# Samsung/tf-fast-rnnt

Hardware: AMD Instinct MI355X
Metric: rnnt_loss_pruned_fwd_bwd_throughput (higher is better)
Workload: dtype f32; 1 GPU; c3: rnnt_loss_pruned fwd+bwd step, B=32/GPU T=1000 S=200 C=500 s_range=5, regular, full boundary, first pass rnnt_loss_simple; global_batch=32, am_pruned=broadcast view

## Files before the change

### tf-fast-rnnt_amd/csrc/prune.hip

```cpp
#include "ftr_common.h"
#include "launch.h"
#include "act_math.h"
#include <cstdlib>
#include <limits.h>

namespace ftr {
namespace {

__device__ __forceinline__ int wave_incl_min_scan(int v, int lane) {
#pragma unroll
  for (int off = 1; off < 64; off <<= 1) {
    const int t = __shfl_up(v, off, 64);
    if (lane >= off) v = min(v, t);
  }
  return v;
}

__global__ void cummin_kernel(const int32_t* __restrict__ in, int32_t* __restrict__ out, int rows, int cols) {
  const int lane = threadIdx.x & 63;
  const int row = blockIdx.x * (blockDim.x >> 6) + (threadIdx.x >> 6);
  if (row >= rows) return;
  const int32_t* src = in + (size_t)row * cols;
  int32_t* dst = out + (size_t)row * cols;
  int carry = INT_MAX;
// ... 13 lines not shown
  const int t = blockIdx.x * blockDim.x + threadIdx.x;
  const int b = blockIdx.y;
  if (t >= T) return;
  const int S1 = S + 1;
  const int nwin = S1 - r + 1;
  const float* pyc = py_grad + (size_t)b * S1 * T + t;
  const float* pxc = px_grad + (size_t)b * S * T1 + t;
  float lead = 0.0f, lag = 0.0f;
  for (int s = 0; s < r; ++s) lead = lead + pyc[(size_t)s * T];
  int best = 0;
  float bestv = 0.0f;
  constexpr int CHK = 16;
  float ld[2][CHK], lg[2][CHK], xv[2][CHK];
  auto fetch = [&](int c0, float (&l)[CHK], float (&g)[CHK], float (&x)[CHK]) {
#pragma unroll
    for (int u = 0; u < CHK; ++u) {
      const int s0 = c0 + u;
      const bool more = s0 + 1 < nwin;
      l[u] = more ? pyc[(size_t)(s0 + r) * T] : 0.0f;
      g[u] = more ? pyc[(size_t)s0 * T] : 0.0f;
      x[u] = (s0 > 0 && s0 < nwin) ? pxc[(size_t)(s0 - 1) * T1] : 0.0f;
    }
  };
  auto consume = [&](int c0, const float (&l)[CHK], const float (&g)[CHK], const float (&x)[CHK]) {
#pragma unroll
    for (int u = 0; u < CHK; ++u) {
      const int s0 = c0 + u;
      if (s0 < nwin) {
        const float blk = lead - lag;
        const float fin = blk - x[u];
        if (s0 == 0 || fin > bestv) { best = s0; bestv = fin; }
        if (s0 + 1 < nwin) {
          lead = lead + l[u];
          lag = lag + g[u];
        }
      }
    }
  };
  fetch(0, ld[0], lg[0], xv[0]);
  for (int c0 = 0; c0 < nwin; c0 += 2 * CHK) {
    if (c0 + CHK < nwin) fetch(c0 + CHK, ld[1], lg[1], xv[1]);
    consume(c0, ld[0], lg[0], xv[0]);
    if (c0 + CHK < nwin) {
      if (c0 + 2 * CHK < nwin) fetch(c0 + 2 * CHK, ld[0], lg[0], xv[0]);
      consume(c0 + CHK, ld[1], lg[1], xv[1]);
    }
  }
  const int se = boundary[4 * b + 2], te = boundary[4 * b + 3];
  int pad = se - r + 1;
  if (pad < 0) pad = 0;
  s_begin[(size_t)b * T + t] = (t < te - 1) ? best : pad;
}

constexpr int kSplitQ = 64;
__global__ __launch_bounds__(512) void prune_argmax_split_kernel(const float* __restrict__ px_grad, const float* __restrict__ py_grad,
                                                                 const int32_t* __restrict__ boundary, int32_t* __restrict__ s_begin,
                                                                 int B, int S, int T, int T1, int r) {
  __shared__ float st_lead[64], st_lag[64], st_bestv[64];
  __shared__ int st_best[64];
  const int lane = threadIdx.x & 63, wave = threadIdx.x >> 6, NW = blockDim.x >> 6;
  const int t = blockIdx.x * 64 + lane;
  const int b = blockIdx.y;
  const bool live = t < T;
  const int tc = live ? t : T - 1;
  const int S1 = S + 1;
  const int nwin = S1 - r + 1;
  const float* pyc = py_grad + (size_t)b * S1 * T + tc;
  const float* pxc = px_grad + (size_t)b * S * T1 + tc;
  constexpr int Q = kSplitQ;
  const int NC = (nwin + Q - 1) / Q;
  float n[Q], g[Q], x[Q];
  auto fetch = [&](int c) {
    const int c0 = c * Q;
#pragma unroll
    for (int u = 0; u < Q; ++u) {
      const int s0 = c0 + u;
      const bool more = s0 + 1 < nwin;
      n[u] = more ? pyc[(size_t)(s0 + r) * T] : 0.0f;
      g[u] = more ? pyc[(size_t)s0 * T] : 0.0f;
      x[u] = (s0 > 0 && s0 < nwin) ? pxc[(size_t)(s0 - 1) * T1] : 0.0f;
    }
  };
  if (wave < NC) fetch(wave);
  float lead = 0.0f, lag = 0.0f, bestv = 0.0f;
  int best = 0;
  if (wave == 0)
    for (int s = 0; s < r; ++s) lead = lead + pyc[(size_t)s * T];
  for (int c = 0; c < NC; ++c) {
    if (c % NW == wave) {
      if (c > 0) { lead = st_lead[lane]; lag = st_lag[lane]; bestv = st_bestv[lane]; best = st_best[lane]; }
      const int c0 = c * Q;
#pragma unroll
      for (int u = 0; u < Q; ++u) {
        const int s0 = c0 + u;
        if (s0 < nwin) {
          const float blk = lead - lag;
          const float fin = blk - x[u];
          if (s0 == 0 || fin > bestv) { best = s0; bestv = fin; }
          if (s0 + 1 < nwin) {
            lead = lead + n[u];
            lag = lag + g[u];
          }
        }
      }
      if (c + 1 < NC) { st_lead[lane] = lead; st_lag[lane] = lag; st_bestv[lane] = bestv; st_best[lane] = best; }
      if (c + NW < NC) fetch(c + NW);
      if (c + 1 == NC && live) {
        const int se = boundary[4 * b + 2], te = boundary[4 * b + 3];
        int pad = se - r + 1;
        if (pad < 0) pad = 0;
        s_begin[(size_t)b * T + t] = (t < te - 1) ? best : pad;
      }
    }
    if (c + 1 < NC) __syncthreads();
  }
}

constexpr int kPruneChk = 64;
template <int R>
__global__ __launch_bounds__(64) void prune_argmax_once_kernel(const float* __restrict__ px_grad, const float* __restrict__ py_grad,
                                         const int32_t* __restrict__ boundary, int32_t* __restrict__ s_begin,
                                         int B, int S, int T, int T1) {
  const int t = blockIdx.x * blockDim.x + threadIdx.x;
  const int b = blockIdx.y;
  if (t >= T) return;
  const int S1 = S + 1;
  const int nwin = S1 - R + 1;
  const float* pyc = py_grad + (size_t)b * S1 * T + t;
  const float* pxc = px_grad + (size_t)b * S * T1 + t;
  constexpr int CHK = kPruneChk;
  float carry[R];
  float lead = 0.0f, lag = 0.0f;
#pragma unroll
  for (int s = 0; s < R; ++s) { carry[s] = pyc[(size_t)s * T]; }
#pragma unroll
  for (int s = 0; s < R; ++s) lead = lead + carry[s];
  int best = 0;
  float bestv = 0.0f;
  float nv[2][CHK], xv[2][CHK];
  auto fetch = [&](int c0, float (&n)[CHK], float (&x)[CHK]) {
#pragma unroll
    for (int u = 0; u < CHK; ++u) {
      const int s0 = c0 + u;
      n[u] = (s0 + 1 < nwin) ? pyc[(size_t)(s0 + R) * T] : 0.0f;
      x[u] = (s0 > 0 && s0 < nwin) ? pxc[(size_t)(s0 - 1) * T1] : 0.0f;
    }
  };
  auto consume = [&](int c0, const float (&n)[CHK], const float (&x)[CHK]) {
#pragma unroll
    for (int u = 0; u < CHK; ++u) {
      const int s0 = c0 + u;
      const float g = (u < R) ? carry[u < R ? u : 0] : n[u >= R ? u - R : 0];
      if (s0 < nwin) {
        const float blk = lead - lag;
        const float fin = blk - x[u];
        if (s0 == 0 || fin > bestv) { best = s0; bestv = fin; }
        if (s0 + 1 < nwin) {
          lead = lead + n[u];
          lag = lag + g;
        }
      }
    }
#pragma unroll
    for (int i = 0; i < R; ++i) carry[i] = n[CHK - R + i];
  };
  fetch(0, nv[0], xv[0]);
  for (int c0 = 0; c0 < nwin; c0 += 2 * CHK) {
    if (c0 + CHK < nwin) fetch(c0 + CHK, nv[1], xv[1]);
    consume(c0, nv[0], xv[0]);
    if (c0 + CHK < nwin) {
      if (c0 + 2 * CHK < nwin) fetch(c0 + 2 * CHK, nv[0], xv[0]);
      consume(c0 + CHK, nv[1], xv[1]);
    }
  }
  const int se = boundary[4 * b + 2], te = boundary[4 * b + 3];
  int pad = se - R + 1;
  if (pad < 0) pad = 0;
  s_begin[(size_t)b * T + t] = (t < te - 1) ? best : pad;
}

__device__ __forceinline__ int wave_incl_suffix_min(int v, int lane) {
#pragma unroll
  for (int off = 1; off < 64; off <<= 1) {
    const int t = __shfl_down(v, off, 64);
    if (lane + off < 64) v = min(v, t);
  }
  return v;
}

__global__ void prune_adjust_kernel(const int32_t* __restrict__ s_begin, int32_t* __restrict__ ranges, int B,
                                    int T, int r_out, int r_con) {
  const int lane = threadIdx.x & 63;
  const int b = blockIdx.x * (blockDim.x >> 6) + (threadIdx.x >> 6);
  if (b >= B) return;
  constexpr int PER = 16, SB = 64 * PER;
  const int32_t* x = s_begin + (size_t)b * T;
  int carry1 = INT_MAX, carry2 = INT_MAX;
  for (int base = ((T - 1) / SB) * SB; base >= 0; base -= SB) {
    const int t0 = base + lane * PER;
    int v[PER];
#pragma unroll
    for (int i = 0; i < PER; ++i) v[i] = (t0 + i < T) ? x[t0 + i] : INT_MAX;
#pragma unroll
    for (int i = PER - 2; i >= 0; --i) v[i] = min(v[i], v[i + 1]);
    int incl = wave_incl_suffix_min(v[0], lane);
    int right = __shfl_down(incl, 1, 64);
    right = (lane == 63) ? carry1 : min(right, carry1);
    carry1 = min(__shfl(incl, 0, 64), carry1);
#pragma unroll
    for (int i = 0; i < PER; ++i) {
      const int t = t0 + i;
      v[i] = (t < T) ? -(min(v[i], right) - (r_con - 1) * t) : INT_MAX;
    }
#pragma unroll
    for (int i = PER - 2; i >= 0; --i) v[i] = min(v[i], v[i + 1]);
    incl = wave_incl_suffix_min(v[0], lane);
    right = __shfl_down(incl, 1, 64);
    right = (lane == 63) ? carry2 : min(right, carry2);
    carry2 = min(__shfl(incl, 0, 64), carry2);
#pragma unroll
    for (int i = 0; i < PER; ++i) {
      const int t = t0 + i;
      if (t < T) {
        const int z = max(min(v[i], right), 0);
        const int sb = -(z - (r_con - 1) * t);
        int32_t* dst = ranges + ((size_t)b * T + t) * r_out;
        for (int k = 0; k < r_out; ++k) dst[k] = sb + k;
      }
    }
  }
}

template <bool VEC>
__global__ __launch_bounds__(128) void do_pruning_kernel(const float* __restrict__ am, const float* __restrict__ lm,
                                                         const int32_t* __restrict__ ranges, float* __restrict__ am_p,
                                                         float* __restrict__ lm_p, int T, int S1, int C, int r) {
  const bool copy_am = am_p != nullptr;
  size_t bt = blockIdx.x;
  if ((gridDim.x & 7u) == 0) bt = (size_t)(blockIdx.x & 7u) * (gridDim.x >> 3) + (blockIdx.x >> 3);
  const size_t b = bt / T;
  const int32_t* rg = ranges + bt * r;
  const float* lmb = lm + b * S1 * C;
  float* ao = am_p + bt * r * C;
  float* lo = lm_p + bt * r * C;
  if (VEC) {
    const int n4 = C >> 2;
    const f4u* arow = reinterpret_cast<const f4u*>(am + bt * C);
    for (int c4 = threadIdx.x; c4 < n4; c4 += 128) {
      f4 a = {0.0f, 0.0f, 0.0f, 0.0f};
      if (copy_am) a = arow[c4];
      for (int k0 = 0; k0 < r; k0 += 8) {
        f4 l[8];
#pragma unroll
        for (int u = 0; u < 8; ++u)
          if (k0 + u < r) l[u] = reinterpret_cast<const f4u*>(lmb + (size_t)min(max(rg[k0 + u], 0), S1 - 1) * C)[c4];
#pragma unroll
        for (int u = 0; u < 8; ++u)
          if (k0 + u < r) {
            if (copy_am) __builtin_nontemporal_store(a, reinterpret_cast<f4u*>(ao + (size_t)(k0 + u) * C) + c4);
            __builtin_nontemporal_store(l[u], reinterpret_cast<f4u*>(lo + (size_t)(k0 + u) * C) + c4);
          }
      }
    }
  } else {
    for (int c = threadIdx.x; c < C; c += 128) {
      const float a = copy_am ? am[bt * C + c] : 0.0f;
      for (int k = 0; k < r; ++k) {
        if (copy_am) ao[(size_t)k * C + c] = a;
        lo[(size_t)k * C + c] = lmb[(size_t)min(max(rg[k], 0), S1 - 1) * C + c];
      }
    }
  }
// ... 1325 lines not shown
    constexpr auto kernel = joiner_act_bwd_lm_kernel<E, ACT, decltype(v)::value>;
    const int rcl = reserve_lds<kernel>(lds, "do_pruning_bwd", LdsText::reserve_why);
    if (rcl != FTR_OK) return rcl;
    hipLaunchKernelGGL(kernel, dim3(S1, B), dim3(64), lds, st, g, y, ranges, d_lm, T, S1, C, r);
    return check_launch("do_pruning_bwd_lm");
  });
}
template <typename E, int ACT>
int joiner_act_bwd_routes(const E* g, const E* y, const int32_t* ranges, E* d_am, E* d_lm, int B, int T, int S1, int C, int r,
                          void* ws, size_t ws_bytes, hipStream_t st) {
  if ((size_t)B * T * C == 0) return FTR_OK;
  const bool vec = bwd_vec4(C, g, y, d_am, d_lm);
  if (!vec || r <= 0) return joiner_act_bwd_generic<E, ACT>(g, y, ranges, d_am, d_lm, B, T, S1, C, r, vec, st);
  const size_t need = do_pruning_bwd_workspace_bytes(B, T, S1, C, r);
  if (!ws || ws_bytes < need || (reinterpret_cast<uintptr_t>(ws) & 15) != 0) {
    set_error("do_pruning_bwd_ws: workspace of %zu bytes (16-byte aligned) required, got %zu", need, ws_bytes);
    return FTR_ERR_INVALID_ARG;
  }
  const int seg = seg_frames(B, T);
  const int nseg = (T + seg - 1) / seg;
  float* partial = reinterpret_cast<float*>(ws);
  int4* meta = reinterpret_cast<int4*>(partial + (size_t)B * nseg * (2 * (size_t)r) * C);
  const size_t lds = sizeof(int) * (size_t)seg;
  if (r > kSegMaxR || lds > 60 * 1024 || (size_t)B * nseg * (2 * (size_t)r) >= 0x7fffffffull || (size_t)B * T * r >= 0x7fffffffull)
    return joiner_act_bwd_generic<E, ACT>(g, y, ranges, d_am, d_lm, B, T, S1, C, r, vec, st);
  dispatch_range<1, kSegMaxR>(r, [&](auto rr) {
    hipLaunchKernelGGL((joiner_act_bwd_seg_kernel<E, ACT, decltype(rr)::value>), dim3(nseg, B), dim3(128), lds, st, g, y, ranges, d_am, d_lm, partial, meta, T, S1, C, seg);
  }, [] {});
  int rc = check_launch("do_pruning_bwd_seg");
  if (rc != FTR_OK) return rc;
  hipLaunchKernelGGL((joiner_act_bwd_reduce_kernel<E, ACT>), dim3(S1, B), dim3(64 * RED_WAVES),
                     sizeof(int) * (size_t)((2 * nseg + 3) & ~3) + 3 * 256 * sizeof(float) * 4, st, g, y, ranges, partial, meta, d_lm, T, S1, C, r, seg, nseg);
  return check_launch("do_pruning_bwd_reduce");
}

}

int do_pruning_bwd(const float* g_am_p, const float* g_lm_p, const int32_t* ranges, float* d_am, float* d_lm, int B,
                   int T, int S1, int C, int r, hipStream_t st) {
  return ftr::do_pruning_bwd_generic(g_am_p, g_lm_p, ranges, d_am, d_lm, B, T, S1, C, r, st);
}

int cummin_i32(const int32_t* in, int32_t* out, int rows, int cols, hipStream_t st) {
  if (rows == 0 || cols == 0) return FTR_OK;
  const int waves_per_block = 4;
  hipLaunchKernelGGL(cummin_kernel, dim3((rows + waves_per_block - 1) / waves_per_block),
                     dim3(64 * waves_per_block), 0, st, in, out, rows, cols);
  return check_launch("cummin_i32");
}

int prune_ranges(const float* px_grad, const float* py_grad, const int32_t* boundary, int32_t* ranges,
                 int32_t* s_begin, int B, int S, int T, int T1, int r, hipStream_t st) {
  if (B == 0 || T == 0) return FTR_OK;
  const int threads = 64;
  const dim3 grid((T + threads - 1) / threads, B);
  const int nwin = S + 1 - r + 1;
  if (nwin > ftr::kSplitQ && (size_t)((T + 63) / 64) * B <= 768) {
    const int nc = (nwin + ftr::kSplitQ - 1) / ftr::kSplitQ;
    const int nw = nc < 8 ? nc : 8;
    hipLaunchKernelGGL(prune_argmax_split_kernel, dim3((T + 63) / 64, B), dim3(64 * nw), 0, st, px_grad, py_grad, boundary, s_begin, B, S, T, T1, r);
  } else
    dispatch_range<1, 16>(r,
      [&](auto rr) { hipLaunchKernelGGL(prune_argmax_once_kernel<decltype(rr)::value>, grid, dim3(threads), 0, st, px_grad, py_grad, boundary, s_begin, B, S, T, T1); },
      [&] { hipLaunchKernelGGL(prune_argmax_kernel, grid, dim3(threads), 0, st, px_grad, py_grad, boundary, s_begin, B, S, T, T1, r); });
  int rc = check_launch("prune_argmax");
  if (rc != FTR_OK) return rc;
  const int r_con = (T1 == T) ? 2 : r;
  hipLaunchKernelGGL(prune_adjust_kernel, dim3(B), dim3(64), 0, st, s_begin, ranges, B, T, r, r_con);
  return check_launch("prune_adjust");
}

int do_pruning(const float* am, const float* lm, const int32_t* ranges, float* am_p, float* lm_p, int B, int T, int S1,
               int C, int r, hipStream_t st) {
  const size_t frames = (size_t)B * T;
  if (frames == 0 || C == 0 || r == 0) return FTR_OK;
  { const int rc32 = require_rows_32bit("do_pruning", frames * (size_t)r); if (rc32 != FTR_OK) return rc32; }
  dispatch((C & 3) == 0, [&](auto vec) {
    hipLaunchKernelGGL(do_pruning_kernel<decltype(vec)::value>, dim3((unsigned)frames), dim3(128), 0, st, am, lm, ranges, am_p, lm_p, T, S1, C, r);
  });
  return check_launch("do_pruning");
}

size_t do_pruning_bwd_workspace_bytes(int B, int T, int S1, int C, int r) {
  if ((C & 3) != 0 || (size_t)B * T * C == 0 || r <= 0) return 0;
  const int seg = ftr::seg_frames(B, T);
  const size_t nseg = (size_t)(T + seg - 1) / seg;
  const size_t partial = sizeof(float) * (size_t)B * nseg * (2 * (size_t)r) * C;
  return partial + sizeof(int4) * (size_t)B * nseg;
}

int do_pruning_bwd_ws(const float* g_am_p, const float* g_lm_p, const int32_t* ranges, float* d_am, float* d_lm,
                      int B, int T, int S1, int C, int r, void* ws, size_t ws_bytes, hipStream_t st) {
  return ftr::do_pruning_bwd_routes(g_am_p, g_lm_p, ranges, d_am, d_lm, B, T, S1, C, r, ws, ws_bytes, st);
}

int do_pruning_sum(const void* am, const void* lm, int dtype, const int32_t* ranges, void* out, int B, int T, int S1, int C,
                   int r, hipStream_t st) {
  const size_t frames = (size_t)B * T;
  if (frames == 0 || C == 0 || r == 0) return FTR_OK;
  { const int rc32 = require_rows_32bit("do_pruning_sum", frames * (size_t)r); if (rc32 != FTR_OK) return rc32; }
  dispatch_dtype(dtype, [&](auto tag) {
    using E = typename decltype(tag)::type;
    dispatch(rows_vec4<E>(C, am, lm) && rows_vec4<E>(C, out), [&](auto vec) {
      hipLaunchKernelGGL((ftr::do_pruning_sum_kernel<E, decltype(vec)::value>), dim3((unsigned)frames), dim3(128), 0, st, static_cast<const E*>(am),
                         static_cast<const E*>(lm), ranges, static_cast<E*>(out), T, S1, C, r);
    });
  });
  return check_launch("do_pruning_sum");
}

int do_pruning_sum_bwd_ws(const void* g, int dtype, const int32_t* ranges, void* d_am, void* d_lm, int B, int T, int S1, int C,
                          int r, void* ws, size_t ws_bytes, hipStream_t st) {
  return dispatch_dtype(dtype, [&](auto tag) {
    using E = typename decltype(tag)::type;
    const E* ge = static_cast<const E*>(g);
    return ftr::do_pruning_bwd_routes(ge, ge, ranges, static_cast<E*>(d_am), static_cast<E*>(d_lm), B, T, S1, C, r, ws, ws_bytes, st);
  });
}

template <typename F>
static inline auto dispatch_act(int act, F&& f) {
// ... 34 lines not shown
```

### tf-fast-rnnt_amd/csrc/simple_fused.hip

```cpp
#include "ftr_common.h"
#include "launch.h"
#include <cstdlib>

namespace ftr {
namespace {

constexpr float kTinyF = 1.401298464324817e-45f;
template <int MB> struct FusedTile {
  static constexpr int FT = 64 * MB, FK = 32, FLD = FK + 4, NBUF = MB == 1 ? 2 : 1;
};
typedef float v4f __attribute__((ext_vector_type(4)));

constexpr int kGLD = 68;
template <int NS, int MB>
__host__ __device__ constexpr size_t fused_lds_bytes() {
  constexpr size_t tile = FusedTile<MB>::NBUF * (size_t)(FusedTile<MB>::FT + 16 * NS) * FusedTile<MB>::FLD;
  constexpr size_t gather = (size_t)16 * NS * kGLD + 16 * NS + (size_t)16 * NS * 8 + (size_t)FusedTile<MB>::FT * 4;
  return sizeof(float) * (tile > gather ? tile : gather);
}

template <bool MOD, bool SMOOTH, int NS, int MB>
__global__ __launch_bounds__(256, 2) void simple_fused_fwd_kernel(
    const float* __restrict__ am, const float* __restrict__ lm, const int32_t* __restrict__ symbols,
    const float* __restrict__ am_probs, const float* __restrict__ lm_probs, const float* __restrict__ am_max,
// ... 194 lines not shown
      const f4 fr = *reinterpret_cast<const f4*>(frec + 4 * (64 * m + 16 * wave + 4 * (lane >> 4) + j));
      amx[j] = fr[0]; a_blank[j] = fr[1]; aon[j] = fr[2];
      pen[j] = (delay_penalty > 0.0) ? (float)((((double)te - 1.0) / 2.0 - (double)t) * delay_penalty) : 0.0f;
    }
    f4 a_sym[NS];
#pragma unroll
    for (int i = 0; i < NS; ++i) a_sym[i] = *reinterpret_cast<const f4*>(asym + (16 * i + n) * kGLD + 16 * wave + 4 * (lane >> 4));
#pragma unroll
    for (int i = 0; i < NS; ++i) {
      const int s = s0 + 16 * i + n;
      if (s > S) continue;
      f4 vy, vx, vp;
#pragma unroll
      for (int j = 0; j < 4; ++j) {
        const int t = tq + j;
        const float pr = acc[m][i][j];
        vp[j] = pr;
        const float nrm = logf(pr + kTinyF) + lmx[i] + amx[j];
        float y = a_blank[j] + lm_blank[i] - nrm;
        if (SMOOTH) y = y * cs + (lm_blank[i] - lon[i]) * ls + (a_blank[j] + ulog_blank - aon[j]) * as;
        vy[j] = y;
        float x = -INFINITY;
        if (s < S && t < T && (MOD || t != te)) {
          x = a_sym[i][j] + lm_sym[i] - nrm;
          if (SMOOTH) x = x * cs + (lm_sym[i] - lon[i]) * ls + (a_sym[i][j] + ulog_sym[i] - aon[j]) * as;
        }
        if (delay_penalty > 0.0) x += pen[j];
        vx[j] = x;
      }
      float* yrow = py + ((size_t)b * (S + 1) + s) * T + tq;
      if (tq + 3 < T) *reinterpret_cast<f4u*>(yrow) = vy;
      else { for (int j = 0; j < 4; ++j) if (tq + j < T) yrow[j] = vy[j]; }
      if (prod_out) {
        float* prow = prod_out + ((size_t)b * (S + 1) + s) * T + tq;
        if (tq + 3 < T) *reinterpret_cast<f4u*>(prow) = vp;
        else { for (int j = 0; j < 4; ++j) if (tq + j < T) prow[j] = vp[j]; }
      }
      if (s < S) {
        float* xrow = px + ((size_t)b * S + s) * T1 + tq;
        if (tq + 3 < T1) *reinterpret_cast<f4u*>(xrow) = vx;
        else { for (int j = 0; j < 4; ++j) if (tq + j < T1) xrow[j] = vx[j]; }
      }
    }
  }
}


constexpr int kBT = 64;
constexpr int kBS = 16;
constexpr int kBLT = kBT + 4;
constexpr int kBCB = 16;

template <int NCB>
__host__ __device__ constexpr size_t fused_bwd_lds_bytes() {
  return sizeof(float) * (2 * kBS * (16 * NCB) + 2 * kBS * kBLT + 2 * kBS * kBT);
}

template <bool MOD, bool USEW, int NCB>
__global__ __launch_bounds__(256, NCB <= 8 ? 4 : 3) void simple_fused_bwd_am_kernel(
    const float* __restrict__ gpx, const float* __restrict__ gpy, const Scale scale, const float* __restrict__ prod,
    const float* __restrict__ lm_probs, const float* __restrict__ am_probs, const int32_t* __restrict__ symbols,
    const int32_t* __restrict__ boundary, int blank, float cs, float kdir, const float* __restrict__ uvec,
    const float* __restrict__ amdot, float as, float* __restrict__ Rout, float* __restrict__ d_am, int T, int S, int C,
    const int32_t* __restrict__ live) {
  extern __shared__ __attribute__((aligned(16))) float smem[];
  constexpr int CT = 16 * NCB, LDC = CT, NG = NCB / 4;
  static_assert(NCB % 4 == 0 && NCB >= 8 && NCB <= 16, "column blocks come in interleaved groups of four");
  float* lmT = smem;
  float* wT = lmT + 2 * kBS * LDC;
  float* csb = wT + 2 * kBS * kBLT;
  int bx = blockIdx.x, by = blockIdx.y, bz = blockIdx.z;
  {
    const unsigned total = gridDim.x * gridDim.y * gridDim.z;
    if ((total & 7u) == 0) {
      const unsigned lin = blockIdx.x + gridDim.x * (blockIdx.y + gridDim.y * blockIdx.z);
      const unsigned j = (lin & 7u) * (total >> 3) + (lin >> 3);
      by = j % gridDim.y; bx = (j / gridDim.y) % gridDim.x; bz = j / (gridDim.x * gridDim.y);
    }
  }
  const int b = bz, t0 = bx * kBT, c0 = by * CT;
  const int tid = threadIdx.x, lane = tid & 63;
  const int wave = __builtin_amdgcn_readfirstlane(tid >> 6);
  const int T1 = MOD ? T : T + 1;
  const int te = boundary ? boundary[4 * b + 3] : T;
  const float sc = scale.at(b);
  const float* gxb = gpx + (size_t)b * S * T1;
  const float* gyb = gpy + (size_t)b * (S + 1) * T;
  const float* prb = prod + (size_t)b * (S + 1) * T;
  const float* lmb = lm_probs + (size_t)b * (S + 1) * C;
  const int nk = (S + 1 + kBS - 1) / kBS;
  int kc_lo = 0, kc_hi = nk;
  if (live) {
    const int32_t* lv = live + (size_t)b * (S + 1) * 2;
    int smin = S + 1, smax = -1;
    for (int s = tid; s <= S; s += 256) {
      const int2 iv = *reinterpret_cast<const int2*>(lv + 2 * s);
      if (iv.x < t0 + kBT && iv.y > t0) { smin = min(smin, s); smax = s; }
    }
    smin = -wave_max_int_dpp(-smin); smax = wave_max_int_dpp(smax);
    int* red = reinterpret_cast<int*>(csb);
    if (lane == 0) { red[wave] = smin; red[4 + wave] = smax; }
    __syncthreads();
    smin = min(min(red[0], red[1]), min(red[2], red[3]));
    smax = max(max(red[4], red[5]), max(red[6], red[7]));
    smin = __builtin_amdgcn_readfirstlane(smin); smax = __builtin_amdgcn_readfirstlane(smax);
    kc_lo = smax < 0 ? 0 : smin / kBS;
    kc_hi = smax < 0 ? 0 : smax / kBS + 1;
    __syncthreads();
  }

  constexpr int NL = (kBS * CT / 4) / 256;
  int lrow[NL], lcol[NL];
  float lmask[NL];
#pragma unroll
  for (int u = 0; u < NL; ++u) {
    const int e = tid + 256 * u, c = c0 + 4 * (e % (CT / 4));
    lrow[u] = e / (CT / 4);
    lcol[u] = min(c, C - 4);
    lmask[u] = c < C ? 1.0f : 0.0f;
  }
  const int wrow = tid >> 4, wq = tid & 15, wt = t0 + 4 * wq;
  const int wtc = min(wt, T - 4);
  const float tmask = wt < T ? 1.0f : 0.0f;
  f4 xmask;
#pragma unroll
  for (int e = 0; e < 4; ++e) xmask[e] = (wt < T && (MOD || wt + e != te)) ? sc : 0.0f;
  const bool want_y = !USEW || uvec != nullptr || (blank >= c0 && blank < c0 + CT);
  const bool want_x = !USEW || uvec != nullptr;
  struct Stage { f4 lv[NL]; f4 x, y, pr; };
  auto load = [&](int kc, Stage& g, bool want_all) {
    const int s = kc * kBS + wrow;
    const int sy_ = min(s, S), sx_ = min(s, S > 0 ? S - 1 : 0);
    if (want_all) {
#pragma unroll
      for (int u = 0; u < NL; ++u) g.lv[u] = *reinterpret_cast<const f4*>(lmb + (size_t)min(kc * kBS + lrow[u], S) * C + lcol[u]);
      g.pr = *reinterpret_cast<const f4u*>(prb + (size_t)sy_ * T + wtc);
      if (want_y) g.y = *reinterpret_cast<const f4u*>(gyb + (size_t)sy_ * T + wtc);
    }
    if (want_x) g.x = (S > 0) ? (f4)*reinterpret_cast<const f4u*>(gxb + (size_t)sx_ * T1 + wtc) : f4{0.f, 0.f, 0.f, 0.f};
  };
  f4 sx = {0.f, 0.f, 0.f, 0.f}, sy = {0.f, 0.f, 0.f, 0.f};

  v4f acc[NCB];
#pragma unroll
  for (int i = 0; i < NCB; ++i) acc[i] = v4f{0.f, 0.f, 0.f, 0.f};
  const int fk = lane >> 4, fn = lane & 15;

  {
    auto park = [&](int kc, const Stage& g) {
      const int buf = kc & 1;
#pragma unroll
      for (int u = 0; u < NL; ++u) {
        const float m = (kc * kBS + lrow[u] <= S) ? lmask[u] : 0.0f;
        *reinterpret_cast<f4*>(lmT + (buf * kBS + lrow[u]) * LDC + 4 * ((tid + 256 * u) % (CT / 4))) = g.lv[u] * m;
      }
      const int s = kc * kBS + wrow;
      const float rowy = s <= S ? sc * tmask : 0.0f, rowx = s < S ? 1.0f : 0.0f;
      f4 w;
      if (USEW) {
        w = (s <= S && wt < T) ? g.pr : f4{0.f, 0.f, 0.f, 0.f};
        if (want_x) sx += g.x * xmask * rowx;
        if (want_y) sy += g.y * rowy;
      } else {
        const f4 x = g.x * xmask * rowx, y = g.y * rowy;
#pragma unroll
        for (int e = 0; e < 4; ++e) w[e] = -cs * (x[e] + y[e]) / (g.pr[e] + kTinyF);
        sx += x; sy += y;
      }
      *reinterpret_cast<f4*>(wT + (buf * kBS + wrow) * kBLT + 4 * wq) = w;
    };
    auto compute = [&](int kc) {
      const int buf = kc & 1;
      const float* abase = lmT + (buf * kBS + fk) * LDC + 4 * fn;
      const float* bbase = wT + (buf * kBS + fk) * kBLT + 16 * wave + fn;
      f4 af[2][NG];
      float bw[kBS / 4];
#pragma unroll
      for (int kk = 0; kk < kBS / 4; ++kk) bw[kk] = bbase[4 * kk * kBLT];
#pragma unroll
      for (int g = 0; g < NG; ++g) af[0][g] = *reinterpret_cast<const f4*>(abase + 64 * g);
#pragma unroll
      for (int kk = 0; kk < kBS / 4; ++kk) {
        if (kk + 1 < kBS / 4) {
#pragma unroll
          for (int g = 0; g < NG; ++g) af[(kk + 1) & 1][g] = *reinterpret_cast<const f4*>(abase + 4 * (kk + 1) * LDC + 64 * g);
        }
        __builtin_amdgcn_sched_barrier(0);
#pragma unroll
        for (int g = 0; g < NG; ++g)
#pragma unroll
          for (int e = 0; e < 4; ++e)
            acc[4 * g + e] = __builtin_amdgcn_mfma_f32_16x16x4f32(af[kk & 1][g][e], bw[kk], acc[4 * g + e], 0, 0, 0);
        __builtin_amdgcn_sched_barrier(0);
      }
    };
    if (kc_lo < kc_hi) {
      Stage g;
      load(kc_lo, g, true);
      park(kc_lo, g);
      __syncthreads();
      for (int kc = kc_lo; kc < kc_hi; ++kc) {
        if (kc + 1 < kc_hi) load(kc + 1, g, true);
        compute(kc);
        if (kc + 1 < kc_hi) park(kc + 1, g);
        __syncthreads();
      }
    }
  }
  *reinterpret_cast<f4*>(csb + (0 * kBS + wrow) * kBT + 4 * wq) = sx;
  *reinterpret_cast<f4*>(csb + (1 * kBS + wrow) * kBT + 4 * wq) = sy;
  __syncthreads();
  const int tl = 16 * wave + fn, t = t0 + tl;
  float cx = 0.0f, cy = 0.0f;
#pragma unroll
  for (int r8 = 0; r8 < kBS; ++r8) { cx += csb[(0 * kBS + r8) * kBT + tl]; cy += csb[(1 * kBS + r8) * kBT + tl]; }
  const bool tok = t < T;
  float R = 0.0f;
  if (uvec && tok) {
    R = -as * (cx + cy) / amdot[(size_t)b * T + t];
    if (by == 0 && fk == 0) Rout[(size_t)b * T + t] = R;
  }
  const float* aprow = am_probs + ((size_t)b * T + (tok ? t : 0)) * C;
#pragma unroll
  for (int g = 0; g < NG; ++g)
#pragma unroll
    for (int j = 0; j < 4; ++j) {
      const int c = c0 + 64 * g + 16 * fk + 4 * j;
      f4 ap = {0.f, 0.f, 0.f, 0.f};
      if (tok && c < C) ap = *reinterpret_cast<const f4*>(aprow + c);
      if (uvec) {
        f4 uv = {0.f, 0.f, 0.f, 0.f};
        if (c < C) uv = *reinterpret_cast<const f4*>(uvec + c);
#pragma unroll
        for (int e = 0; e < 4; ++e) acc[4 * g + e][j] = ap[e] * (acc[4 * g + e][j] + uv[e] * R);
      } else {
#pragma unroll
        for (int e = 0; e < 4; ++e) acc[4 * g + e][j] = ap[e] * acc[4 * g + e][j];
      }
    }
  {
    constexpr int kB2 = CT / 2;
    static_assert(kB2 * kBT <= 2 * kBS * LDC && kB2 <= 2 * kBS * kBLT, "pass 2 reuses the tiles of pass 1");
    float* xT = lmT;
    int* sym2 = reinterpret_cast<int*>(wT);
    constexpr int kCap = (2 * kBS * kBLT - kB2) * 2;
    unsigned short* rlist = reinterpret_cast<unsigned short*>(wT + kB2);
    int* wcnt = reinterpret_cast<int*>(csb);
    int count = 0;
    const bool listed = S <= 65535;
    const int r_lo = min(kc_lo * kBS, S), r_hi = min(kc_hi * kBS, S);
    __syncthreads();
    if (listed) {
      for (int base = r_lo; base < r_hi; base += 256) {
        const int srow = base + tid;
        const int sy = srow < r_hi ? min(max(symbols[(size_t)b * S + srow], 0), C - 1) : -1;
        const bool mine = sy >= c0 && sy < c0 + CT;
        const unsigned long long m = __ballot(mine);
        if (lane == 0) wcnt[wave] = __popcll(m);
        __syncthreads();
        int off = count;
        for (int w = 0; w < wave; ++w) off += wcnt[w];
        const int tot = wcnt[0] + wcnt[1] + wcnt[2] + wcnt[3];
        const int at = off + __popcll(m & ((1ull << lane) - 1ull));
        if (mine && at < kCap) rlist[at] = (unsigned short)srow;
        count += tot;
        __syncthreads();
      }
    }
    const bool all_rows = !listed || count > kCap;
    if (all_rows) count = r_hi - r_lo;
    auto row_of = [&](int i) { return all_rows ? r_lo + i : (int)rlist[i]; };
    constexpr int NX = kB2 * (kBT / 4) / 256;
    for (int r0 = 0; r0 < count; r0 += kB2) {
      f4 xv[NX];
#pragma unroll
      for (int u = 0; u < NX; ++u) {
        const int row = row_of(min(r0 + wrow + 16 * u, count - 1));
        xv[u] = *reinterpret_cast<const f4u*>(gxb + (size_t)row * T1 + wtc);
      }
      const int li = r0 + tid;
      const int symr = (tid < kB2 && li < count) ? min(max(symbols[(size_t)b * S + row_of(li)], 0), C - 1) : -1;
      __syncthreads();
#pragma unroll
      for (int u = 0; u < NX; ++u) {
        const float rowx = (r0 + wrow + 16 * u < count) ? kdir : 0.0f;
        *reinterpret_cast<f4*>(xT + (wrow + 16 * u) * kBT + 4 * wq) = xv[u] * xmask * rowx;
      }
      if (tid < kB2) sym2[tid] = symr;
      __syncthreads();
      const int nks = (min(kB2, count - r0) + 3) / 4;
      for (int kk = 0; kk < nks; ++kk) {
        const float bx = xT[(4 * kk + fk) * kBT + 16 * wave + fn];
        const int lc = sym2[4 * kk + fk] - c0;
        const int myblk = (lc >= 0 && lc < CT && ((lc & 63) >> 2) == fn) ? 4 * (lc >> 6) + (lc & 3) : -1;
        unsigned mask = 0;
#pragma unroll
        for (int q = 0; q < 4; ++q) {
          const int sb = __builtin_amdgcn_readfirstlane(sym2[4 * kk + q]) - c0;
          if (sb >= 0 && sb < CT) mask |= 1u << (4 * (sb >> 6) + (sb & 3));
        }
#pragma unroll
        for (int i = 0; i < NCB; ++i)
          if (mask & (1u << i)) acc[i] = __builtin_amdgcn_mfma_f32_16x16x4f32((myblk == i) ? 1.0f : 0.0f, bx, acc[i], 0, 0, 0);
      }
    }
  }
  if (!tok) return;
  float* drow = d_am + ((size_t)b * T + t) * C;
  const float colb = kdir * cy;
#pragma unroll
  for (int g = 0; g < NG; ++g)
#pragma unroll
    for (int j = 0; j < 4; ++j) {
      const int c = c0 + 64 * g + 16 * fk + 4 * j;
      if (c >= C) continue;
      f4 v = {acc[4 * g + 0][j], acc[4 * g + 1][j], acc[4 * g + 2][j], acc[4 * g + 3][j]};
      if (blank >= c && blank < c + 4) v[blank - c] += colb;
      *reinterpret_cast<f4*>(drow + c) = v;
    }
}

}

int simple_fused_supported(int C) { return (C % 4 == 0) ? 1 : 0; }

int simple_fused_fwd(const float* am, const float* lm, const int32_t* symbols, const float* am_probs,
                     const float* lm_probs, const float* am_max, const float* lm_max, const int32_t* boundary, int blank,
                     double delay_penalty, const float* lmonly_norm, const float* amonly_norm, const float* ulog, float cs,
                     float ls, float as, float* px, float* py, float* prod_out, int B, int T, int S, int C, int modified,
                     hipStream_t st) {
  if (!simple_fused_supported(C)) { set_error("simple_logprobs_fused_fwd: C = %d is not a multiple of 4", C); return FTR_ERR_UNSUPPORTED; }
  const int T1 = modified ? T : T + 1;
  const int blocks = (S + 1 + 15) / 16;
  const int ny = (blocks + 12) / 13;
// ... 80 lines not shown
```

Before: 25600 utterances/s.

## Stage prune argmax through LDS with producer waves and widen adjust kernel

Replaces the split and per-thread prune argmax kernels with a producer/consumer kernel. Four producer waves load py/px gradient rows as vectorized float4 into an LDS ring buffer, and one consumer wave runs the sliding-window argmax out of shared memory. A block-index swizzle is added. The prune_adjust kernel now uses several waves per batch row, combining suffix minima through shared memory. The aim is to replace strided scalar global loads with coalesced vector loads and to raise parallelism in the adjust step, at the cost of a __syncthreads per chunk and a single consumer wave per tile.

```diff
diff --git a/tf-fast-rnnt_amd/csrc/prune.hip b/tf-fast-rnnt_amd/csrc/prune.hip
--- a/tf-fast-rnnt_amd/csrc/prune.hip
+++ b/tf-fast-rnnt_amd/csrc/prune.hip
@@ -89,131 +89,117 @@
   s_begin[(size_t)b * T + t] = (t < te - 1) ? best : pad;
 }
 
-constexpr int kSplitQ = 64;
-__global__ __launch_bounds__(512) void prune_argmax_split_kernel(const float* __restrict__ px_grad, const float* __restrict__ py_grad,
-                                                                 const int32_t* __restrict__ boundary, int32_t* __restrict__ s_begin,
-                                                                 int B, int S, int T, int T1, int r) {
-  __shared__ float st_lead[64], st_lag[64], st_bestv[64];
-  __shared__ int st_best[64];
-  const int lane = threadIdx.x & 63, wave = threadIdx.x >> 6, NW = blockDim.x >> 6;
-  const int t = blockIdx.x * 64 + lane;
-  const int b = blockIdx.y;
-  const bool live = t < T;
-  const int tc = live ? t : T - 1;
+constexpr int kStageQ = 16;
+constexpr int kStageRing = 4;
+constexpr int kStageDepth = 2;
+constexpr int kStageProd = 4;
+constexpr int kStageMaxR = 16;
+static_assert(kStageMaxR <= kStageQ && (kStageRing & (kStageRing - 1)) == 0 && kStageRing >= 3, "the lag rows must lie in the chunk before");
+
+template <bool VEC>
+__device__ __forceinline__ f4 stage_load4(const float* __restrict__ row, int col, int T) {
+  if (VEC) return *reinterpret_cast<const f4u*>(row + min(col, T - 4));
+  f4 v;
+  v.x = row[min(col, T - 1)]; v.y = row[min(col + 1, T - 1)]; v.z = row[min(col + 2, T - 1)]; v.w = row[min(col + 3, T - 1)];
+  return v;
+}
+
+template <bool VEC>
+__global__ __launch_bounds__(64 * (1 + kStageProd)) void prune_argmax_staged_kernel(const float* __restrict__ px_grad, const float* __restrict__ py_grad,
+                                                                                  const int32_t* __restrict__ boundary, int32_t* __restrict__ s_begin,
+                                                                                  int S, int T, int T1, int r, int tiles) {
+  constexpr int Q = kStageQ, D = kStageDepth, NP = 64 * kStageProd;
+  constexpr int PER = Q * 16 / NP;
+  constexpr int RMASK = kStageRing * Q - 1;
+  static_assert(PER * NP == Q * 16, "a chunk must divide among the producer threads");
+  __shared__ __attribute__((aligned(16))) float py_s[kStageRing * Q * 64];
+  __shared__ __attribute__((aligned(16))) float px_s[2 * Q * 64];
+  const int lane = threadIdx.x & 63;
+  const bool producer = threadIdx.x >= 64;
+  const int pi = (int)threadIdx.x - 64;
+  unsigned id = blockIdx.x;
+  if ((gridDim.x & 7u) == 0) id = (blockIdx.x & 7u) * (gridDim.x >> 3) + (blockIdx.x >> 3);
+  const int b = (int)(id / (unsigned)tiles);
+  const int t0 = (int)(id % (unsigned)tiles) * 64;
   const int S1 = S + 1;
-  const int nwin = S1 - r + 1;
-  const float* pyc = py_grad + (size_t)b * S1 * T + tc;
-  const float* pxc = px_grad + (size_t)b * S * T1 + tc;
-  constexpr int Q = kSplitQ;
-  const int NC = (nwin + Q - 1) / Q;
-  float n[Q], g[Q], x[Q];
-  auto fetch = [&](int c) {
-    const int c0 = c * Q;
-#pragma unroll
-    for (int u = 0; u < Q; ++u) {
-      const int s0 = c0 + u;
-      const bool more = s0 + 1 < nwin;
-      n[u] = more ? pyc[(size_t)(s0 + r) * T] : 0.0f;
-      g[u] = more ? pyc[(size_t)s0 * T] : 0.0f;
-      x[u] = (s0 > 0 && s0 < nwin) ? pxc[(size_t)(s0 - 1) * T1] : 0.0f;
+  const int NC = (S + 2 + Q - 1) / Q;
+  const float* pyb = py_grad + (size_t)b * S1 * T;
+  const float* pxb = px_grad + (size_t)b * S * T1;
+  f4 ry[D][PER], rx[D][PER];
+  auto fetch = [&](int c, f4 (&y)[PER], f4 (&x)[PER]) {
+#pragma unroll
+    for (int u = 0; u < PER; ++u) {
+      const int i = pi + u * NP;
+      const int row = c * Q + (i >> 4), col = t0 + 4 * (i & 15);
+      y[u] = stage_load4<VEC>(pyb + (size_t)min(row, S) * T, col, T);
+      x[u] = stage_load4<VEC>(pxb + (size_t)min(max(row - r - 1, 0), S - 1) * T1, col, T);
     }
   };
-  if (wave < NC) fetch(wave);
+  auto put = [&](int c, const f4 (&y)[PER], const f4 (&x)[PER]) {
+#pragma unroll
+    for (int u = 0; u < PER; ++u) {
+      const int i = pi + u * NP;
+      const int xrow = c * Q + (i >> 4) - r - 1;
+      const float neutral = (xrow == -1) ? 0.0f : __builtin_inff();
+      const bool none = xrow < 0 || xrow > S - r;
+      f4 xv = x[u];
+      xv.x = none ? neutral : xv.x; xv.y = none ? neutral : xv.y; xv.z = none ? neutral : xv.z; xv.w = none ? neutral : xv.w;
+      *reinterpret_cast<f4*>(py_s + (((c * Q + (i >> 4)) & RMASK) * 64 + 4 * (i & 15))) = y[u];
+      *reinterpret_cast<f4*>(px_s + (((c & 1) * Q + (i >> 4)) * 64 + 4 * (i & 15))) = xv;
+    }
+  };
   float lead = 0.0f, lag = 0.0f, bestv = 0.0f;
   int best = 0;
-  if (wave == 0)
-    for (int s = 0; s < r; ++s) lead = lead + pyc[(size_t)s * T];
-  for (int c = 0; c < NC; ++c) {
-    if (c % NW == wave) {
-      if (c > 0) { lead = st_lead[lane]; lag = st_lag[lane]; bestv = st_bestv[lane]; best = st_best[lane]; }
-      const int c0 = c * Q;
-#pragma unroll
-      for (int u = 0; u < Q; ++u) {
-        const int s0 = c0 + u;
-        if (s0 < nwin) {
-          const float blk = lead - lag;
-          const float fin = blk - x[u];
-          if (s0 == 0 || fin > bestv) { best = s0; bestv = fin; }
-          if (s0 + 1 < nwin) {
-            lead = lead + n[u];
-            lag = lag + g[u];
-          }
-        }
-      }
-      if (c + 1 < NC) { st_lead[lane] = lead; st_lag[lane] = lag; st_bestv[lane] = bestv; st_best[lane] = best; }
-      if (c + NW < NC) fetch(c + NW);
-      if (c + 1 == NC && live) {
-        const int se = boundary[4 * b + 2], te = boundary[4 * b + 3];
-        int pad = se - r + 1;
-        if (pad < 0) pad = 0;
-        s_begin[(size_t)b * T + t] = (t < te - 1) ? best : pad;
-      }
-    }
-    if (c + 1 < NC) __syncthreads();
-  }
-}
-
-constexpr int kPruneChk = 64;
-template <int R>
-__global__ __launch_bounds__(64) void prune_argmax_once_kernel(const float* __restrict__ px_grad, const float* __restrict__ py_grad,
-                                         const int32_t* __restrict__ boundary, int32_t* __restrict__ s_begin,
-                                         int B, int S, int T, int T1) {
-  const int t = blockIdx.x * blockDim.x + threadIdx.x;
-  const int b = blockIdx.y;
-  if (t >= T) return;
-  const int S1 = S + 1;
-  const int nwin = S1 - R + 1;
-  const float* pyc = py_grad + (size_t)b * S1 * T + t;
-  const float* pxc = px_grad + (size_t)b * S * T1 + t;
-  constexpr int CHK = kPruneChk;
-  float carry[R];
-  float lead = 0.0f, lag = 0.0f;
-#pragma unroll
-  for (int s = 0; s < R; ++s) { carry[s] = pyc[(size_t)s * T]; }
-#pragma unroll
-  for (int s = 0; s < R; ++s) lead = lead + carry[s];
-  int best = 0;
-  float bestv = 0.0f;
-  float nv[2][CHK], xv[2][CHK];
-  auto fetch = [&](int c0, float (&n)[CHK], float (&x)[CHK]) {
-#pragma unroll
-    for (int u = 0; u < CHK; ++u) {
-      const int s0 = c0 + u;
-      n[u] = (s0 + 1 < nwin) ? pyc[(size_t)(s0 + R) * T] : 0.0f;
-      x[u] = (s0 > 0 && s0 < nwin) ? pxc[(size_t)(s0 - 1) * T1] : 0.0f;
+  auto consume = [&](int c) {
+    float n[Q], g[Q], x[Q];
+#pragma unroll
+    for (int u = 0; u < Q; ++u) {
+      const int p = c * Q + u;
+      n[u] = py_s[(p & RMASK) * 64 + lane];
+      g[u] = py_s[((p - r) & RMASK) * 64 + lane];
+      x[u] = px_s[((c & 1) * Q + u) * 64 + lane];
+    }
+#pragma unroll
+    for (int u = 0; u < Q; ++u) {
+      const int s0 = c * Q + u - r;
+      const float blk = lead - lag;
+      const float fin = blk - x[u];
+      const bool take = (fin > bestv) | (s0 == 0);
+      best = take ? s0 : best;
+      bestv = take ? fin : bestv;
+      lead = lead + n[u];
+      lag = lag + g[u];
     }
   };
-  auto consume = [&](int c0, const float (&n)[CHK], const float (&x)[CHK]) {
-#pragma unroll
-    for (int u = 0; u < CHK; ++u) {
-      const int s0 = c0 + u;
-      const float g = (u < R) ? carry[u < R ? u : 0] : n[u >= R ? u - R : 0];
-      if (s0 < nwin) {
-        const float blk = lead - lag;
-        const float fin = blk - x[u];
-        if (s0 == 0 || fin > bestv) { best = s0; bestv = fin; }
-        if (s0 + 1 < nwin) {
-          lead = lead + n[u];
-          lag = lag + g;
-        }
-      }
-    }
-#pragma unroll
-    for (int i = 0; i < R; ++i) carry[i] = n[CHK - R + i];
-  };
-  fetch(0, nv[0], xv[0]);
-  for (int c0 = 0; c0 < nwin; c0 += 2 * CHK) {
-    if (c0 + CHK < nwin) fetch(c0 + CHK, nv[1], xv[1]);
-    consume(c0, nv[0], xv[0]);
-    if (c0 + CHK < nwin) {
-      if (c0 + 2 * CHK < nwin) fetch(c0 + 2 * CHK, nv[0], xv[0]);
-      consume(c0 + CHK, nv[1], xv[1]);
-    }
-  }
-  const int se = boundary[4 * b + 2], te = boundary[4 * b + 3];
-  int pad = se - R + 1;
-  if (pad < 0) pad = 0;
-  s_begin[(size_t)b * T + t] = (t < te - 1) ? best : pad;
+  static_assert(kStageMaxR * 16 <= NP, "one 16-byte piece of the zero rows per producer thread");
+  if (producer && pi < kStageMaxR * 16)
+    *reinterpret_cast<f4*>(py_s + ((RMASK + 1 - kStageMaxR) * 64 + 4 * pi)) = f4{0.0f, 0.0f, 0.0f, 0.0f};
+  if (producer) {
+#pragma unroll
+    for (int d = 0; d < D; ++d)
+      if (d < NC) fetch(d, ry[d], rx[d]);
+  }
+  for (int c0 = 0; c0 < NC; c0 += D) {
+#pragma unroll
+    for (int d = 0; d < D; ++d) {
+      const int c = c0 + d;
+      if (c < NC) {
+        if (producer) {
+          put(c, ry[d], rx[d]);
+          if (c + D < NC) fetch(c + D, ry[d], rx[d]);
+        }
+        __syncthreads();
+        if (!producer) consume(c);
+      }
+    }
+  }
+  const int t = t0 + lane;
+  if (!producer && t < T) {
+    const int se = boundary[4 * b + 2], te = boundary[4 * b + 3];
+    int pad = se - r + 1;
+    if (pad < 0) pad = 0;
+    s_begin[(size_t)b * T + t] = (t < te - 1) ? best : pad;
+  }
 }
 
 __device__ __forceinline__ int wave_incl_suffix_min(int v, int lane) {
@@ -225,25 +211,44 @@
   return v;
 }
 
-__global__ void prune_adjust_kernel(const int32_t* __restrict__ s_begin, int32_t* __restrict__ ranges, int B,
-                                    int T, int r_out, int r_con) {
-  const int lane = threadIdx.x & 63;
-  const int b = blockIdx.x * (blockDim.x >> 6) + (threadIdx.x >> 6);
-  if (b >= B) return;
-  constexpr int PER = 16, SB = 64 * PER;
+constexpr int kAdjustPer = 16;
+constexpr int kAdjustMaxWaves = 16;
+
+__device__ __forceinline__ int adjust_right_min(int first, int lane, int wave, int nw, int* tot, int& carry) {
+  const int incl = wave_incl_suffix_min(first, lane);
+  int right = __shfl_down(incl, 1, 64);
+  right = (lane == 63) ? carry : min(right, carry);
+  int all = __shfl(incl, 0, 64);
+  if (nw > 1) {
+    if (lane == 0) tot[wave] = all;
+    __syncthreads();
+    for (int w = 0; w < nw; ++w) {
+      const int v = tot[w];
+      if (w > wave) right = min(right, v);
+      all = min(all, v);
+    }
+  }
+  carry = min(all, carry);
+  return right;
+}
+
+__global__ __launch_bounds__(64 * kAdjustMaxWaves) void prune_adjust_kernel(const int32_t* __restrict__ s_begin, int32_t* __restrict__ ranges,
+                                                                            int T, int r_out, int r_con) {
+  __shared__ int tot[2][kAdjustMaxWaves];
+  const int lane = threadIdx.x & 63, wave = threadIdx.x >> 6, nw = blockDim.x >> 6;
+  const int b = blockIdx.x;
+  constexpr int PER = kAdjustPer;
+  const int SB = (int)blockDim.x * PER;
   const int32_t* x = s_begin + (size_t)b * T;
   int carry1 = INT_MAX, carry2 = INT_MAX;
   for (int base = ((T - 1) / SB) * SB; base >= 0; base -= SB) {
-    const int t0 = base + lane * PER;
+    const int t0 = base + (int)threadIdx.x * PER;
     int v[PER];
 #pragma unroll
     for (int i = 0; i < PER; ++i) v[i] = (t0 + i < T) ? x[t0 + i] : INT_MAX;
 #pragma unroll
     for (int i = PER - 2; i >= 0; --i) v[i] = min(v[i], v[i + 1]);
-    int incl = wave_incl_suffix_min(v[0], lane);
-    int right = __shfl_down(incl, 1, 64);
-    right = (lane == 63) ? carry1 : min(right, carry1);
-    carry1 = min(__shfl(incl, 0, 64), carry1);
+    int right = adjust_right_min(v[0], lane, wave, nw, tot[0], carry1);
 #pragma unroll
     for (int i = 0; i < PER; ++i) {
       const int t = t0 + i;
@@ -251,10 +256,7 @@
     }
 #pragma unroll
     for (int i = PER - 2; i >= 0; --i) v[i] = min(v[i], v[i + 1]);
-    incl = wave_incl_suffix_min(v[0], lane);
-    right = __shfl_down(incl, 1, 64);
-    right = (lane == 63) ? carry2 : min(right, carry2);
-    carry2 = min(__shfl(incl, 0, 64), carry2);
+    right = adjust_right_min(v[0], lane, wave, nw, tot[1], carry2);
 #pragma unroll
     for (int i = 0; i < PER; ++i) {
       const int t = t0 + i;
@@ -1686,21 +1688,22 @@
 int prune_ranges(const float* px_grad, const float* py_grad, const int32_t* boundary, int32_t* ranges,
                  int32_t* s_begin, int B, int S, int T, int T1, int r, hipStream_t st) {
   if (B == 0 || T == 0) return FTR_OK;
-  const int threads = 64;
-  const dim3 grid((T + threads - 1) / threads, B);
-  const int nwin = S + 1 - r + 1;
-  if (nwin > ftr::kSplitQ && (size_t)((T + 63) / 64) * B <= 768) {
-    const int nc = (nwin + ftr::kSplitQ - 1) / ftr::kSplitQ;
-    const int nw = nc < 8 ? nc : 8;
-    hipLaunchKernelGGL(prune_argmax_split_kernel, dim3((T + 63) / 64, B), dim3(64 * nw), 0, st, px_grad, py_grad, boundary, s_begin, B, S, T, T1, r);
-  } else
-    dispatch_range<1, 16>(r,
-      [&](auto rr) { hipLaunchKernelGGL(prune_argmax_once_kernel<decltype(rr)::value>, grid, dim3(threads), 0, st, px_grad, py_grad, boundary, s_begin, B, S, T, T1); },
-      [&] { hipLaunchKernelGGL(prune_argmax_kernel, grid, dim3(threads), 0, st, px_grad, py_grad, boundary, s_begin, B, S, T, T1, r); });
+  const size_t tiles = (size_t)(T + 63) / 64;
+  if (r <= ftr::kStageMaxR && tiles * B <= 0x7fffffffull) {
+    dispatch((T & 3) == 0, [&](auto vec) {
+      hipLaunchKernelGGL(ftr::prune_argmax_staged_kernel<decltype(vec)::value>, dim3((unsigned)(tiles * B)), dim3(64 * (1 + ftr::kStageProd)), 0, st,
+                         px_grad, py_grad, boundary, s_begin, S, T, T1, r, (int)tiles);
+    });
+  } else {
+    const int threads = 64;
+    hipLaunchKernelGGL(prune_argmax_kernel, dim3((T + threads - 1) / threads, B), dim3(threads), 0, st, px_grad, py_grad, boundary, s_begin, B, S, T, T1, r);
+  }
   int rc = check_launch("prune_argmax");
   if (rc != FTR_OK) return rc;
   const int r_con = (T1 == T) ? 2 : r;
-  hipLaunchKernelGGL(prune_adjust_kernel, dim3(B), dim3(64), 0, st, s_begin, ranges, B, T, r, r_con);
+  const int per_wave = 64 * ftr::kAdjustPer;
+  const int waves = (T + per_wave - 1) / per_wave < ftr::kAdjustMaxWaves ? (T + per_wave - 1) / per_wave : ftr::kAdjustMaxWaves;
+  hipLaunchKernelGGL(prune_adjust_kernel, dim3(B), dim3(64 * waves), 0, st, s_begin, ranges, T, r, r_con);
   return check_launch("prune_adjust");
 }
 
```

Measured after the change: 25580 utterances/s, median of 3. No clear change (-0.1%).

## Build symbol row list during GEMM pass and prefetch am_probs and x early

Applied to the files above, without the earlier changes.

Moves the per-column-block symbol row list construction out of the second pass and into the first-pass pipeline, with a dedicated LDS region plus cached column offsets for narrow tiles. For NCB<=8, the loop is restructured so that the last compute step runs after the am_probs row, the amdot value and the first gpx rows have been issued, hiding their latency behind MFMA work. Column sums now reuse an lm buffer, one barrier is dropped, and the symbol global re-reads in pass 2 are replaced by rcol lookups. The cost is more register pressure from holding ap and xv across compute, plus a changed LDS footprint that may affect occupancy.

```diff
diff --git a/tf-fast-rnnt_amd/csrc/simple_fused.hip b/tf-fast-rnnt_amd/csrc/simple_fused.hip
--- a/tf-fast-rnnt_amd/csrc/simple_fused.hip
+++ b/tf-fast-rnnt_amd/csrc/simple_fused.hip
@@ -270,8 +270,10 @@
 constexpr int kBCB = 16;
 
 template <int NCB>
+__host__ __device__ constexpr int fused_bwd_list_cap() { return (2 * kBS * kBLT - 8 * NCB) * 2; }
+template <int NCB>
 __host__ __device__ constexpr size_t fused_bwd_lds_bytes() {
-  return sizeof(float) * (2 * kBS * (16 * NCB) + 2 * kBS * kBLT + 2 * kBS * kBT);
+  return sizeof(float) * (2 * kBS * (16 * NCB) + 2 * kBS * kBLT) + (NCB <= 8 ? 3 : 2) * (size_t)fused_bwd_list_cap<NCB>() + 12 * sizeof(int);
 }
 
 template <bool MOD, bool USEW, int NCB>
@@ -286,7 +288,12 @@
   static_assert(NCB % 4 == 0 && NCB >= 8 && NCB <= 16, "column blocks come in interleaved groups of four");
   float* lmT = smem;
   float* wT = lmT + 2 * kBS * LDC;
-  float* csb = wT + 2 * kBS * kBLT;
+  constexpr int kCap = fused_bwd_list_cap<NCB>();
+  unsigned short* rlist = reinterpret_cast<unsigned short*>(wT + 2 * kBS * kBLT);
+  constexpr bool kCols = NCB <= 8;
+  unsigned char* rcol = reinterpret_cast<unsigned char*>(rlist + kCap);
+  int* red = reinterpret_cast<int*>(rcol + (kCols ? kCap : 0));
+  static_assert(2 * kBS * kBT <= kBS * LDC, "the column sums fit one lm buffer");
   int bx = blockIdx.x, by = blockIdx.y, bz = blockIdx.z;
   {
     const unsigned total = gridDim.x * gridDim.y * gridDim.z;
@@ -307,6 +314,9 @@
   const float* prb = prod + (size_t)b * (S + 1) * T;
   const float* lmb = lm_probs + (size_t)b * (S + 1) * C;
   const int nk = (S + 1 + kBS - 1) / kBS;
+  const int32_t* symb = symbols + (size_t)b * S;
+  int sym0 = -1;
+  if (S > 0) sym0 = symb[min(tid, S - 1)];
   int kc_lo = 0, kc_hi = nk;
   if (live) {
     const int32_t* lv = live + (size_t)b * (S + 1) * 2;
@@ -316,7 +326,6 @@
       if (iv.x < t0 + kBT && iv.y > t0) { smin = min(smin, s); smax = s; }
     }
     smin = -wave_max_int_dpp(-smin); smax = wave_max_int_dpp(smax);
-    int* red = reinterpret_cast<int*>(csb);
     if (lane == 0) { red[wave] = smin; red[4 + wave] = smax; }
     __syncthreads();
     smin = min(min(red[0], red[1]), min(red[2], red[3]));
@@ -324,7 +333,6 @@
     smin = __builtin_amdgcn_readfirstlane(smin); smax = __builtin_amdgcn_readfirstlane(smax);
     kc_lo = smax < 0 ? 0 : smin / kBS;
     kc_hi = smax < 0 ? 0 : smax / kBS + 1;
-    __syncthreads();
   }
 
   constexpr int NL = (kBS * CT / 4) / 256;
@@ -363,6 +371,62 @@
 #pragma unroll
   for (int i = 0; i < NCB; ++i) acc[i] = v4f{0.f, 0.f, 0.f, 0.f};
   const int fk = lane >> 4, fn = lane & 15;
+
+  constexpr int kB2 = CT / 2;
+  static_assert(kCap == (2 * kBS * kBLT - kB2) * 2, "list capacity");
+  int count = 0;
+  const bool listed = S <= 65535;
+  const int r_lo = min(kc_lo * kBS, S), r_hi = min(kc_hi * kBS, S);
+  auto build_list = [&]() {
+    if (!listed) return;
+    int* wcnt = red + 8;
+    for (int base = r_lo & ~255; base < r_hi; base += 256) {
+      const int srow = base + tid;
+      const int raw = base == 0 ? sym0 : symb[min(srow, S - 1)];
+      const int sy = (srow >= r_lo && srow < r_hi) ? min(max(raw, 0), C - 1) : -1;
+      const bool mine = sy >= c0 && sy < c0 + CT;
+      const unsigned long long m = __ballot(mine);
+      if (lane == 0) wcnt[wave] = __popcll(m);
+      __syncthreads();
+      int off = count;
+      for (int w = 0; w < wave; ++w) off += wcnt[w];
+      const int tot = wcnt[0] + wcnt[1] + wcnt[2] + wcnt[3];
+      const int at = off + __popcll(m & ((1ull << lane) - 1ull));
+      if (mine && at < kCap) { rlist[at] = (unsigned short)srow; if (kCols) rcol[at] = (unsigned char)(sy - c0); }
+      count += __builtin_amdgcn_readfirstlane(tot);
+      __syncthreads();
+    }
+  };
+  f4 ap[NG][4];
+  float adot = 1.0f;
+  auto fetch_ap = [&]() {
+    const int t = t0 + 16 * wave + fn;
+    const float* aprow = am_probs + ((size_t)b * T + (t < T ? t : 0)) * C;
+#pragma unroll
+    for (int g = 0; g < NG; ++g)
+#pragma unroll
+      for (int j = 0; j < 4; ++j) ap[g][j] = *reinterpret_cast<const f4*>(aprow + min(c0 + 64 * g + 16 * fk + 4 * j, C - 4));
+    if (uvec) adot = amdot[(size_t)b * T + (t < T ? t : 0)];
+  };
+  constexpr int NX = kB2 * (kBT / 4) / 256;
+  f4 xv[NX];
+  bool all_rows = false;
+  auto fetch_x = [&](int r0) {
+#pragma unroll
+    for (int u = 0; u < NX; ++u) {
+      const int i = max(min(r0 + wrow + 16 * u, count - 1), 0);
+      const int row = all_rows ? r_lo + i : (int)rlist[i];
+      xv[u] = *reinterpret_cast<const f4u*>(gxb + (size_t)row * T1 + wtc);
+    }
+  };
+  auto fetch_x_first = [&]() {
+#pragma unroll
+    for (int u = 0; u < NX; ++u) {
+      const int row = min((int)rlist[max(min(wrow + 16 * u, min(count, kCap) - 1), 0)], S - 1);
+      xv[u] = *reinterpret_cast<const f4u*>(gxb + (size_t)row * T1 + wtc);
+    }
+  };
+  constexpr bool kEarly = NCB <= 8;
 
   {
     auto park = [&](int kc, const Stage& g) {
@@ -414,90 +478,68 @@
     };
     if (kc_lo < kc_hi) {
       Stage g;
+      if (!kEarly) build_list();
       load(kc_lo, g, true);
+      if (kEarly) build_list();
       park(kc_lo, g);
       __syncthreads();
-      for (int kc = kc_lo; kc < kc_hi; ++kc) {
-        if (kc + 1 < kc_hi) load(kc + 1, g, true);
+      for (int kc = kc_lo; kc + (kEarly ? 1 : 0) < kc_hi; ++kc) {
+        const bool more = kEarly || kc + 1 < kc_hi;
+        if (more) load(kc + 1, g, true);
         compute(kc);
-        if (kc + 1 < kc_hi) park(kc + 1, g);
+        if (more) park(kc + 1, g);
         __syncthreads();
       }
     }
-  }
+    all_rows = !listed || count > kCap;
+    if (all_rows) count = r_hi - r_lo;
+    if (kEarly) fetch_ap();
+    if (kEarly && kc_lo < kc_hi) compute(kc_hi - 1);
+    if (kEarly && S > 0) fetch_x_first();
+  }
+  const int tl = 16 * wave + fn, t = t0 + tl;
+  const bool tok = t < T;
+  const float* aprow = am_probs + ((size_t)b * T + (tok ? t : 0)) * C;
+  float* csb = lmT + (kc_hi & 1) * kBS * LDC;
   *reinterpret_cast<f4*>(csb + (0 * kBS + wrow) * kBT + 4 * wq) = sx;
   *reinterpret_cast<f4*>(csb + (1 * kBS + wrow) * kBT + 4 * wq) = sy;
   __syncthreads();
-  const int tl = 16 * wave + fn, t = t0 + tl;
   float cx = 0.0f, cy = 0.0f;
 #pragma unroll
   for (int r8 = 0; r8 < kBS; ++r8) { cx += csb[(0 * kBS + r8) * kBT + tl]; cy += csb[(1 * kBS + r8) * kBT + tl]; }
-  const bool tok = t < T;
   float R = 0.0f;
   if (uvec && tok) {
-    R = -as * (cx + cy) / amdot[(size_t)b * T + t];
+    R = -as * (cx + cy) / (kEarly ? adot : amdot[(size_t)b * T + t]);
     if (by == 0 && fk == 0) Rout[(size_t)b * T + t] = R;
   }
-  const float* aprow = am_probs + ((size_t)b * T + (tok ? t : 0)) * C;
 #pragma unroll
   for (int g = 0; g < NG; ++g)
 #pragma unroll
     for (int j = 0; j < 4; ++j) {
       const int c = c0 + 64 * g + 16 * fk + 4 * j;
-      f4 ap = {0.f, 0.f, 0.f, 0.f};
-      if (tok && c < C) ap = *reinterpret_cast<const f4*>(aprow + c);
+      f4 apq = {0.f, 0.f, 0.f, 0.f};
+      if (kEarly) { if (tok && c < C) apq = ap[g][j]; }
+      else if (tok && c < C) apq = *reinterpret_cast<const f4*>(aprow + c);
       if (uvec) {
         f4 uv = {0.f, 0.f, 0.f, 0.f};
         if (c < C) uv = *reinterpret_cast<const f4*>(uvec + c);
 #pragma unroll
-        for (int e = 0; e < 4; ++e) acc[4 * g + e][j] = ap[e] * (acc[4 * g + e][j] + uv[e] * R);
+        for (int e = 0; e < 4; ++e) acc[4 * g + e][j] = apq[e] * (acc[4 * g + e][j] + uv[e] * R);
       } else {
 #pragma unroll
-        for (int e = 0; e < 4; ++e) acc[4 * g + e][j] = ap[e] * acc[4 * g + e][j];
+        for (int e = 0; e < 4; ++e) acc[4 * g + e][j] = apq[e] * acc[4 * g + e][j];
       }
     }
   {
-    constexpr int kB2 = CT / 2;
     static_assert(kB2 * kBT <= 2 * kBS * LDC && kB2 <= 2 * kBS * kBLT, "pass 2 reuses the tiles of pass 1");
     float* xT = lmT;
     int* sym2 = reinterpret_cast<int*>(wT);
-    constexpr int kCap = (2 * kBS * kBLT - kB2) * 2;
-    unsigned short* rlist = reinterpret_cast<unsigned short*>(wT + kB2);
-    int* wcnt = reinterpret_cast<int*>(csb);
-    int count = 0;
-    const bool listed = S <= 65535;
-    const int r_lo = min(kc_lo * kBS, S), r_hi = min(kc_hi * kBS, S);
-    __syncthreads();
-    if (listed) {
-      for (int base = r_lo; base < r_hi; base += 256) {
-        const int srow = base + tid;
-        const int sy = srow < r_hi ? min(max(symbols[(size_t)b * S + srow], 0), C - 1) : -1;
-        const bool mine = sy >= c0 && sy < c0 + CT;
-        const unsigned long long m = __ballot(mine);
-        if (lane == 0) wcnt[wave] = __popcll(m);
-        __syncthreads();
-        int off = count;
-        for (int w = 0; w < wave; ++w) off += wcnt[w];
-        const int tot = wcnt[0] + wcnt[1] + wcnt[2] + wcnt[3];
-        const int at = off + __popcll(m & ((1ull << lane) - 1ull));
-        if (mine && at < kCap) rlist[at] = (unsigned short)srow;
-        count += tot;
-        __syncthreads();
-      }
-    }
-    const bool all_rows = !listed || count > kCap;
-    if (all_rows) count = r_hi - r_lo;
-    auto row_of = [&](int i) { return all_rows ? r_lo + i : (int)rlist[i]; };
-    constexpr int NX = kB2 * (kBT / 4) / 256;
     for (int r0 = 0; r0 < count; r0 += kB2) {
-      f4 xv[NX];
-#pragma unroll
-      for (int u = 0; u < NX; ++u) {
-        const int row = row_of(min(r0 + wrow + 16 * u, count - 1));
-        xv[u] = *reinterpret_cast<const f4u*>(gxb + (size_t)row * T1 + wtc);
-      }
+      if (r0 > 0 || !kEarly || all_rows) fetch_x(r0);
       const int li = r0 + tid;
-      const int symr = (tid < kB2 && li < count) ? min(max(symbols[(size_t)b * S + row_of(li)], 0), C - 1) : -1;
+      int symr = -1;
+      if (tid < kB2 && li < count)
+        symr = (kCols && !all_rows) ? c0 + (int)rcol[li] : min(max(symb[all_rows ? r_lo + li : (int)rlist[li]], 0), C - 1);
       __syncthreads();
 #pragma unroll
       for (int u = 0; u < NX; ++u) {
```

New measurement: 25500 utterances/s before, 25560 utterances/s after, median of 4. Within noise of the previous version (+0.2%).
